# py-lidbox/lidbox

Hardware: AMD Instinct MI355X
Metric: utterances/sec (16kHz x 2s) log-mel + x-vector train step (higher is better)
Workload: dtype f32; 1 GPU; log-mel + x-vector 4-lang train step, bs=256 per GPU, fp32 (BASELINE configs[1]); reference_model=lidbox.models.xvector, global_batch=256, per_gpu_batch=256, samples_per_utt=32000, frames=198, mel=40, languages=4, optimizer=Adam(1e-3, eps=1e-7), parallelism=dp1, grad_buckets=1, grad_sync=none, hip_graph=True, resident_batches=4, feature_prefetch=False

## Files before the change

lidbox_amd/csrc/gemm.hip:

```cpp
#include <stdlib.h>

#include <atomic>

#include "gemm_shared.h"
#include "gemm_sk.h"
#include <string.h>
#include "gemm_dma.h"
#include "gemm_dma8.h"
#include "gemm_tuned.h"

namespace {

constexpr int BK = 16;
#define LBX_ROWS_BOUNDS(BM, BN) __launch_bounds__(256, ((BM) * (BN) >= 16384 ? 3 : ((BM) * (BN) >= 8192 ? 6 : 8)))
#define LBX_TN_BOUNDS(BM, BN) __launch_bounds__(256, ((BM) * (BN) >= 16384 ? 3 : 1))

template <int ROWS, bool ALIGNED, int NT = 256>
struct KInnerLoader {
    static constexpr int F4R = BK / 4;
    static constexpr int RPP = NT / F4R;
    static constexpr int PASSES = ROWS >= RPP ? ROWS / RPP : 1;
    static constexpr bool PARTIAL = ROWS < RPP;
    static constexpr int LD = ROWS + 8 / F4R;
    float4 v[PASSES];
    const float* ptr[PASSES];
    int c4, r0, k;

    __device__ __forceinline__ void init(const RowsD& rows, long row_base, long nrows, int tid, int kbeg) {
        c4 = tid % F4R;
        r0 = tid / F4R;
        k = kbeg + c4 * 4;
#pragma unroll
        for (int p = 0; p < PASSES; ++p) {
            const long r = row_base + r0 + p * RPP;
            ptr[p] = rows.base + ((r < nrows && !(PARTIAL && r0 >= ROWS)) ? row_offset(rows, (unsigned)r) : 0) + k;
        }
    }
    template <bool CHECK>
    __device__ __forceinline__ void load(int kend) {
#pragma unroll
        for (int p = 0; p < PASSES; ++p) {
            float4 x;
            if (!CHECK) {
                if (ALIGNED) x = *reinterpret_cast<const float4*>(ptr[p]);
                else x = make_float4(ptr[p][0], ptr[p][1], ptr[p][2], ptr[p][3]);
            } else {
                x = make_float4(0.f, 0.f, 0.f, 0.f);
                if (ALIGNED) {
                    if (k < kend) x = *reinterpret_cast<const float4*>(ptr[p]);
                } else {
                    if (k + 0 < kend) x.x = ptr[p][0];
                    if (k + 1 < kend) x.y = ptr[p][1];
                    if (k + 2 < kend) x.z = ptr[p][2];
                    if (k + 3 < kend) x.w = ptr[p][3];
                }
            }
            ptr[p] += BK;
            v[p] = x;
        }
        k += BK;
    }
    __device__ __forceinline__ void store(float* tile) const {
        if (PARTIAL && r0 >= ROWS) return;
#pragma unroll
        for (int p = 0; p < PASSES; ++p) {
            float* d = tile + (c4 * 4) * LD + r0 + p * RPP;
            d[0 * LD] = v[p].x;
            d[1 * LD] = v[p].y;
            d[2 * LD] = v[p].z;
            d[3 * LD] = v[p].w;
        }
    }
};

template <int COLS, bool ALIGNED, int NT = 256>
struct KOuterLoader {
    static constexpr int F4 = COLS / 4;
    static constexpr int RPP = NT / F4;
    static constexpr int PASSES = BK >= RPP ? BK / RPP : 1;
    static constexpr bool PARTIAL = BK < RPP;
    static constexpr int LD = COLS;
    float4 v[PASSES];
    const float* ptr[PASSES];
    long step;
    int c4, kk0, c, cload, kcur, ncols_;

    __device__ __forceinline__ void init(int tid, int col0, int ncols) {
        c4 = tid % F4;
        kk0 = tid / F4;
        if (PARTIAL && kk0 >= BK) kk0 -= BK;
        c = col0 + c4 * 4;
        ncols_ = ncols;
        cload = (ALIGNED && c >= ncols) ? 0 : c;
    }
    __device__ __forceinline__ void init_plain(const float* base, long ld, int kbeg, int col0, int ncols, int tid) {
        init(tid, col0, ncols);
        kcur = kbeg + kk0;
        step = (long)BK * ld;
#pragma unroll
        for (int p = 0; p < PASSES; ++p) ptr[p] = base + (long)(kcur + RPP * p) * ld + cload;
    }
    template <bool CHECK>
    __device__ __forceinline__ void load_plain(int kend) {
#pragma unroll
        for (int p = 0; p < PASSES; ++p) {
            v[p] = fetch<CHECK>(ptr[p], (kcur + RPP * p) < kend);
            ptr[p] += step;
        }
        kcur += BK;
    }
    template <bool CHECK>
    __device__ __forceinline__ void load_rows(const float* base, const long (&off)[PASSES],
                                              const bool (&ok)[PASSES]) {
#pragma unroll
        for (int p = 0; p < PASSES; ++p) v[p] = fetch<CHECK>(base + off[p] + cload, ok[p]);
    }
    template <bool CHECK>
    __device__ __forceinline__ float4 fetch(const float* src, bool row_ok) const {
        float4 x = make_float4(0.f, 0.f, 0.f, 0.f);
        if (ALIGNED) {
            if (!CHECK || row_ok) x = *reinterpret_cast<const float4*>(src);
        } else if (!CHECK || row_ok) {
            if (c + 0 < ncols_) x.x = src[0];
            if (c + 1 < ncols_) x.y = src[1];
            if (c + 2 < ncols_) x.z = src[2];
            if (c + 3 < ncols_) x.w = src[3];
        }
        return x;
    }
    __device__ __forceinline__ void store(float* tile) const {
#pragma unroll
        for (int p = 0; p < PASSES; ++p)
            *reinterpret_cast<float4*>(tile + (kk0 + RPP * p) * LD + c4 * 4) = v[p];
    }
};

template <int MI, int NJ, int LDA, int LDB>
__device__ __forceinline__ void mma_tile(const float* As, const float* Bs, int wm, int wn, int lane,
                                         f32x16 (&acc)[MI][NJ]) {
    const int h = lane >> 5, l = lane & 31;
    const float* ap = As + h * LDA + wm * (32 * MI) + l;
    const float* bp = Bs + h * LDB + wn * (32 * NJ) + l;
    float a[2][MI], b[2][NJ];
    __builtin_amdgcn_s_setprio(3);
#pragma unroll
    for (int i = 0; i < MI; ++i) a[0][i] = ap[32 * i];
#pragma unroll
    for (int j = 0; j < NJ; ++j) b[0][j] = bp[32 * j];
#pragma unroll
    for (int kk = 0; kk < BK; kk += 2) {
        const int cur = (kk >> 1) & 1, nxt = cur ^ 1;
        if (kk + 2 < BK) {
#pragma unroll
            for (int i = 0; i < MI; ++i) a[nxt][i] = ap[(kk + 2) * LDA + 32 * i];
#pragma unroll
            for (int j = 0; j < NJ; ++j) b[nxt][j] = bp[(kk + 2) * LDB + 32 * j];
        }
        __builtin_amdgcn_sched_barrier(0);
#pragma unroll
        for (int i = 0; i < MI; ++i)
#pragma unroll
            for (int j = 0; j < NJ; ++j)
// ... 232 lines not shown

__global__ void colsum_stage2(const float* __restrict__ partial, int slices, int N, float* __restrict__ out,
                              int accumulate) {
    const int c = blockIdx.x * blockDim.x + threadIdx.x;
    if (c >= N) return;
    float s = 0.f;
    for (int k = 0; k < slices; ++k) s += partial[(long)k * N + c];
    out[c] = accumulate ? out[c] + s : s;
}

inline bool sk_enabled() {
    const char* e = getenv("LIDBOX_GEMM_SK");
    return !(e && atoi(e) == 0);
}
inline unsigned sk_grid() {
    if (const char* e = getenv("LIDBOX_GEMM_SK_GRID")) {
        const int g = atoi(e);
        if (g >= 1 && g <= NUM_CU * SK_WGCU) return (unsigned)g;
    }
    return NUM_CU * SK_WGCU;
}
inline double sk_min_flop() {
    if (const char* e = getenv("LIDBOX_GEMM_SK_MIN_FLOP")) return atof(e);
    return 3.0e9;
}
constexpr int SK_MIN_SPAN = 8;
constexpr int SK_PART_STEPS = 16;

inline unsigned sk_next_epoch() {
    static std::atomic<unsigned> e{0};
    unsigned v;
    do v = e.fetch_add(1u) + 1u; while ((v & 0xffffffu) == 0u);
    return v & 0xffffffu;
}

struct SkRows {
    bool ok = false;
    SkPlan pl{};
    unsigned P = 0;
    size_t ws_need = 0;
};

inline bool sk_all() {
    const char* e = getenv("LIDBOX_GEMM_SK_ALL");
    return e && atoi(e) != 0;
}
inline bool sk_rows_policy(int kind, int K) { return sk_all() || (kind == 0 && K >= 1024); }
inline bool sk_tuned_out(int kind, long M, int N, int K) { return !sk_all() && tuned_gemm(kind, M, N, K) != nullptr; }

inline int skp_mode() {
    if (const char* e = getenv("LIDBOX_GEMM_SKP")) return atoi(e);
    return 1;
}

inline bool skp_policy(int kind, long M, int N, int K) {
    (void)kind; (void)M; (void)N; (void)K;
    return skp_mode() == 2;
}

SkRows sk_rows_plan(int kind, long M, int N, int K, bool pipelined = false) {
    SkRows c;
    if (!sk_enabled() || M < SK_BM || K % 4 != 0 || 2.0 * (double)M * N * K < sk_min_flop()) return c;
    if (!pipelined && !sk_rows_policy(kind, K)) return c;
    unsigned P = sk_grid();
    if (pipelined && P == (unsigned)(NUM_CU * SK_WGCU)) P = NUM_CU * SKP_WGCU;
    if (P % 8 != 0) return c;
    SkPlan& pl = c.pl;
    pl.tiles_n = (int)lbx_cdiv(N, SK_BN);
    const long T = lbx_cdiv(M, SK_BM) * pl.tiles_n;
    if (T > 0x3fffffffL) return c;
    pl.ntiles = (int)T;
    pl.nk = (int)lbx_cdiv(K, SK_BK);
    pl.ktail = K - (pl.nk - 1) * SK_BK;
    pl.dp_rounds = (int)(T / P);
    pl.sk_first = pl.dp_rounds * (int)P;
    pl.sk_tiles = (int)T - pl.sk_first;
    pl.parts = 0;
    if (pl.dp_rounds > 0 && pl.sk_tiles > 0) {
        long g = pl.nk / SK_PART_STEPS;
        if (g > (long)(P / 8) / lbx_cdiv(pl.sk_tiles, 8)) g = (long)(P / 8) / lbx_cdiv(pl.sk_tiles, 8);
        if (g < 1) g = 1;
        if (g > 200) g = 200;
        const long wg_cu = P / NUM_CU > 0 ? P / NUM_CU : 1;
        const double cu_parts = (double)pl.dp_rounds * pl.nk * wg_cu + (double)lbx_cdiv(pl.sk_tiles * g, NUM_CU) * ((double)pl.nk / g);
        const double cu_spans = 1.05 * (double)T * pl.nk / NUM_CU;
        if (cu_parts <= cu_spans) {
            pl.parts = (int)g;
        } else {
            --pl.dp_rounds;
            pl.sk_first = pl.dp_rounds * (int)P;
            pl.sk_tiles = (int)T - pl.sk_first;
        }
    }
    if (pl.parts == 0 && pl.sk_tiles > 0 && (long)pl.sk_tiles * pl.nk < (long)P * SK_MIN_SPAN) return c;
    if (pl.parts == 0 && pl.sk_tiles > 0 && (long)pl.nk * P / ((long)pl.sk_tiles * pl.nk) + 2 > 250) return c;
    if ((size_t)pl.sk_tiles * sizeof(unsigned) > SK_COUNTER_BYTES) return c;
    c.P = P;
    c.ws_need = SK_COUNTER_BYTES + (size_t)P * 2 * SK_SLAB * sizeof(float) + (pipelined ? SKP_DUMMY_BYTES : 0);
    c.ok = true;
    return c;
}

inline bool sk_extent_ok(const lidbox_rows_t& r, long cols) {
    const double last = (double)(r.batch > 0 ? r.batch - 1 : 0) * r.batch_stride + (double)(r.rows_per_batch > 0 ? r.rows_per_batch - 1 : 0) * r.row_stride + cols + 64;
    return last * 4.0 < 4.0e9;
}

inline bool sk_b_extent_ok(bool b_kinner, int K, int N, long ldb) {
    return ((double)(b_kinner ? N : K) + 16.0) * (double)ldb * 4.0 < 4.0e9;
}

void sk_set_lds_attr() {
    static const bool done = [] {
        (void)hipFuncSetAttribute((const void*)gemm_sk_rows_kernel<false>, hipFuncAttributeMaxDynamicSharedMemorySize, (int)SK_LDS_BYTES);
        (void)hipFuncSetAttribute((const void*)gemm_sk_rows_kernel<true>, hipFuncAttributeMaxDynamicSharedMemorySize, (int)SK_LDS_BYTES);
        (void)hipFuncSetAttribute((const void*)gemm_sk_tn_kernel, hipFuncAttributeMaxDynamicSharedMemorySize, (int)SK_LDS_BYTES);
#define LBX_SKP_ATTR(B_, M_, A_) (void)hipFuncSetAttribute((const void*)gemm_skp_rows_kernel<B_, M_, A_>, hipFuncAttributeMaxDynamicSharedMemorySize, (int)SKP_LDS_BYTES)
        LBX_SKP_ATTR(false, false, false); LBX_SKP_ATTR(false, true, false); LBX_SKP_ATTR(false, false, true); LBX_SKP_ATTR(false, true, true);
        LBX_SKP_ATTR(true, false, false); LBX_SKP_ATTR(true, true, false); LBX_SKP_ATTR(true, false, true); LBX_SKP_ATTR(true, true, true);
#undef LBX_SKP_ATTR
        return true;
    }();
    (void)done;
}

struct SkTn {
    bool ok = false;
    int splits = 0, tiles_n = 0, ntiles = 0;
    long rows_per_split = 0;
    size_t ws_need = 0;
};

SkTn sk_tn_plan(long M, int K1, int N) {
    SkTn c;
    if (!sk_enabled() || K1 % 4 != 0 || N % 4 != 0 || 2.0 * (double)M * N * K1 < 2.0 * sk_min_flop()) return c;
    c.tiles_n = (int)lbx_cdiv(N, SK_BN);
    c.ntiles = (int)lbx_cdiv(K1, SK_BM) * c.tiles_n;
    long g = (long)sk_grid() / c.ntiles;
    if (g < 1) g = 1;
    long rps = lbx_cdiv(lbx_cdiv(M, g), SK_BK) * SK_BK;
    if (rps < 8 * SK_BK) return c;
    if (rps > 8192) rps = 8192;
    c.rows_per_split = rps;
    c.splits = (int)lbx_cdiv(M, rps);
    c.ws_need = ((size_t)c.splits * K1 * N + (size_t)c.splits * N) * sizeof(float);
    c.ok = true;
    return c;
}

struct RowsChoice {
    int bm, bn, splits, k_per_split;
    bool no_tail_split = false;
    int waves = 4;
};

thread_local int g_last_launches[3] = {0, 0, 0};
thread_local int g_last_family = 0;
thread_local int g_first_tile[2] = {0, 0};
thread_local int g_last_carried = 0;

const int CAND[4][2] = {{128, 128}, {128, 64}, {64, 128}, {64, 64}};
const double TILE_EFF[4] = {1.0, 0.98, 0.97, 0.955};
const int RESIDENT[4] = {3, 4, 4, 6};
const double FIXED_STEPS[4] = {6.0, 5.0, 5.0, 3.0};

inline double conc_eff(double w) {
    if (w <= 1.0) return 0.55;
    if (w <= 2.0) return 0.55 + 0.25 * (w - 1.0);
    if (w <= 3.0) return 0.80 + 0.10 * (w - 2.0);
    return 0.92;
}

inline double launch_cost(int c, long wgs, double ksteps) {
    const int bm = CAND[c][0], bn = CAND[c][1];
    const double tile_t = (bm * bn / 16384.0) * (ksteps + FIXED_STEPS[c]) / TILE_EFF[c];
    double per_cu = (double)lbx_cdiv(wgs, NUM_CU);
    if (wgs > NUM_CU && wgs % NUM_CU != 0) {
        const double fluid = (double)wgs / NUM_CU + 0.12;
        if (fluid < per_cu) per_cu = fluid;
    }
    const double conc = per_cu < RESIDENT[c] ? (double)wgs / NUM_CU : (double)RESIDENT[c];
    return per_cu * tile_t / conc_eff(conc < 1.0 ? 1.0 : conc);
}

RowsChoice choose_rows(int kind, long M, int N, int K, size_t ws_bytes) {
    if (const TunedGemm* t = tuned_gemm(kind, M, N, K)) {
        const int kps = (int)(lbx_cdiv(lbx_cdiv(K, t->splits), BK) * BK);
        const int splits = (int)lbx_cdiv(K, kps);
        if (splits == 1 || (size_t)splits * M * N * sizeof(float) <= ws_bytes)
            return RowsChoice{t->bm, t->bn, splits, kps, t->no_tail_split != 0, (t->waves == 8 && t->bm == 128) ? 8 : 4};
    }
    RowsChoice best{128, 128, 1, K};
    double best_cost = 1e30;
    for (int c = 0; c < 4; ++c) {
        const int bm = CAND[c][0], bn = CAND[c][1];
        const long tiles = lbx_cdiv(M, bm) * lbx_cdiv(N, bn);
        for (int s = 1; s <= 64; s *= 2) {
            int kps = (int)(lbx_cdiv(lbx_cdiv(K, s), BK) * BK);
            const int splits = (int)lbx_cdiv(K, kps);
            if (s > 1 && (splits < 2 || kps < 4 * BK)) break;
            if (splits > 1 && (size_t)splits * M * N * sizeof(float) > ws_bytes) break;
            double cost = launch_cost(c, tiles * splits, (double)kps / BK);
            if (splits > 1) cost += 5.0 + (double)M * N * 4.0 * (splits + 1) / 3.0e6;
            if (cost < best_cost) { best_cost = cost; best = RowsChoice{bm, bn, splits, kps}; }
            if (splits < s) break;
        }
    }
    return best;
}

RowsChoice choose_rows_env(int kind, long M, int N, int K, size_t wsb) {
    RowsChoice ch = choose_rows(kind, M, N, K, wsb);
    if (M >= 4096) {
        if (const char* f = getenv(kind == 1 ? "LIDBOX_GEMM_NT8" : "LIDBOX_GEMM_NN8")) {
            const int bn = atoi(f);
            if (bn == 64 || bn == 128) return RowsChoice{128, bn, 1, K, false, 8};
        }
    }
    if (const char* f = getenv("LIDBOX_GEMM_PLAN")) {
        int bm = 0, bn = 0, sp = 0, wv = 4;
        if (sscanf(f, "%d,%d,%d,%d", &bm, &bn, &sp, &wv) >= 3 && (bm == 64 || bm == 128) && (bn == 64 || bn == 128) && sp >= 1) {
            const int kps = (int)(lbx_cdiv(lbx_cdiv(K, sp), BK) * BK);
            const int splits = (int)lbx_cdiv(K, kps);
            if (splits == 1 || (size_t)splits * M * N * sizeof(float) <= wsb)
                ch = RowsChoice{bm, bn, splits, kps, false, (wv == 8 && bm == 128) ? 8 : 4};
        }
    }
    return ch;
}

template <int BM, int BN, bool B_KINNER>
void launch_rows8_t(bool al, dim3 grid, hipStream_t st, RowsD Ad, const float* Bm, long ldb, RowsOutD Co, float* P,
                    long m_beg, long m_end, int K, int N, int epi, const float* aux, int tiles_n, unsigned ntiles, int kps) {
    if (al)
        hipLaunchKernelGGL((gemm_rows8_kernel<BM, BN, B_KINNER, true>), grid, dim3(512), 0, st, Ad, Bm, ldb, Co, P, m_beg,
                           m_end, K, N, epi, aux, tiles_n, ntiles, kps);
    else
        hipLaunchKernelGGL((gemm_rows8_kernel<BM, BN, B_KINNER, false>), grid, dim3(512), 0, st, Ad, Bm, ldb, Co, P, m_beg,
                           m_end, K, N, epi, aux, tiles_n, ntiles, kps);
}

template <int BM, int BN, bool B_KINNER>
void launch_rows_t(bool al, dim3 grid, hipStream_t st, RowsD Ad, const float* Bm, long ldb, RowsOutD Co, float* P,
                   long m_beg, long m_end, int K, int N, int epi, const float* aux, int tiles_n, unsigned ntiles, int kps) {
    if (al)
        hipLaunchKernelGGL((gemm_rows_kernel<BM, BN, B_KINNER, true>), grid, dim3(256), 0, st, Ad, Bm, ldb, Co, P, m_beg,
                           m_end, K, N, epi, aux, tiles_n, ntiles, kps);
    else
        hipLaunchKernelGGL((gemm_rows_kernel<BM, BN, B_KINNER, false>), grid, dim3(256), 0, st, Ad, Bm, ldb, Co, P, m_beg,
                           m_end, K, N, epi, aux, tiles_n, ntiles, kps);
}

inline int dma_mode() {
    if (const char* e = getenv("LIDBOX_GEMM_DMA")) return atoi(e);
    return 1;
}

template <int BM, int BN, bool B_KINNER>
void launch_rows_dma_t(dim3 grid, hipStream_t st, RowsD Ad, const float* Bm, long ldb, RowsOutD Co, float* P, long m_beg, long m_end,
                       int K, int N, int epi, const float* aux, int tiles_n, unsigned ntiles, int kps, const DmaStream& sp, const ReduceJobs& rj) {
    hipLaunchKernelGGL((gemm_rows_dma_kernel<BM, BN, B_KINNER>), grid, dim3(256), 0, st, Ad, Bm, ldb, Co, P, m_beg, m_end, K, N, epi,
                       aux, tiles_n, ntiles, kps, sp, rj);
}

inline long carry_cap() {
    if (const char* e = getenv("LIDBOX_GEMM_CARRY_BLOCKS")) { const long v = atol(e); if (v >= 8) return v; }
    return 96;
}
struct Carry {
    const ReduceJob* jobs = nullptr;
    int njobs = 0;
    bool carried = false;
};

constexpr int DMA_STREAM_MIN_STEPS = 8;
constexpr int DMA_STREAM_MAX_G = 8;
struct DmaStreamPlan {
    int g = 0;
    long whole = 0, rem = 0;
    size_t ws_need = 0;
};
inline DmaStreamPlan dma_stream_plan(int bm, int bn, long M, int N, int K) {
    DmaStreamPlan pl;
    int force = -1;
    if (const char* e = getenv("LIDBOX_GEMM_STREAM_TAIL")) force = atoi(e);
    if (force == 0) return pl;
    const long tiles = lbx_cdiv(M, bm) * lbx_cdiv(N, bn);
    const long rem = tiles % NUM_CU;
    if (tiles < NUM_CU || rem == 0) return pl;
    const int nk = (int)lbx_cdiv(K, SK_BK);
    int best = 1;
    double best_cost = 1.0;
    for (int g = 2; g <= DMA_STREAM_MAX_G && nk / g >= DMA_STREAM_MIN_STEPS; ++g) {
        const double cost = (double)lbx_cdiv(rem * g, (long)NUM_CU) / g + 0.03 + 0.01 * g;
        if (cost < best_cost - 1e-9) { best_cost = cost; best = g; }
    }
    if (force > 1 && nk / force >= 2 && force <= 64) best = force;
    else if (best_cost > 0.9) return pl;
    if (best < 2) return pl;
    pl.g = best; pl.rem = rem; pl.whole = tiles - rem;
    pl.ws_need = SK_COUNTER_BYTES + (size_t)rem * best * bm * bn * sizeof(float);
    return pl;
}

template <bool B_KINNER>
int launch_rows_range(const RowsChoice& ch, bool al, RowsD Ad, const float* Bm, long ldb, RowsOutD Co, long m_beg,
                      long m_end, int K, int N, int epi, const float* aux, float* P, hipStream_t st, bool dma_ok = false,
                      const DmaStreamPlan* stream = nullptr, void* ws = nullptr, Carry* carry = nullptr) {
    const long Msub = m_end - m_beg;
    if (Msub <= 0) return LIDBOX_OK;
    const int tiles_n = (int)lbx_cdiv(N, ch.bn);
    const long ntiles = lbx_cdiv(Msub, ch.bm) * tiles_n;
    dim3 grid((unsigned)ntiles, (unsigned)ch.splits);
    if (g_last_launches[0] == 0) { g_first_tile[0] = ch.bm; g_first_tile[1] = ch.bn; }
    ++g_last_launches[(ch.bm == g_first_tile[0] && ch.bn == g_first_tile[1]) ? 0 : 1];
    if (ch.splits > 1) ++g_last_launches[2];
#define LBX_ROWS(BM_, BN_) launch_rows_t<BM_, BN_, B_KINNER>(al, grid, st, Ad, Bm, ldb, Co, P, m_beg, m_end, K, N, epi, aux, tiles_n, (unsigned)ntiles, ch.k_per_split)
#define LBX_ROWS8(BM_, BN_) launch_rows8_t<BM_, BN_, B_KINNER>(al, grid, st, Ad, Bm, ldb, Co, P, m_beg, m_end, K, N, epi, aux, tiles_n, (unsigned)ntiles, ch.k_per_split)
#define LBX_ROWS_DMA(BM_, BN_) launch_rows_dma_t<BM_, BN_, B_KINNER>(grid, st, Ad, Bm, ldb, Co, P, m_beg, m_end, K, N, epi, aux, tiles_n, ntiles_k, ch.k_per_split, sp, rj)
    if (dma_ok && al && dma_mode() != 0) {
        g_last_family = 1;
        DmaStream sp;
        const bool dma8 = ch.waves == 8 && ch.bm == 128;
        ReduceJobs rj;
        if (carry && !carry->carried && carry->njobs > 0) {
            rj = pack_carry(carry->jobs, carry->njobs, carry_cap());
            carry->carried = rj.total > 0;
        }
        unsigned ntiles_k = (unsigned)ntiles;
        if (stream && stream->g > 1 && ch.splits == 1) {
            sp.pieces = (unsigned)(stream->rem * stream->g);
            sp.npad = (sp.pieces + 7u) & ~7u;
            sp.g = stream->g;
            sp.first_tile = (unsigned)stream->whole;
            sp.epoch = sk_next_epoch();
            sp.counters = (unsigned*)ws;
            sp.slabs = (float*)((char*)ws + SK_COUNTER_BYTES);
            ntiles_k = (unsigned)stream->whole;
            grid.x = sp.npad + ntiles_k;
        }
        grid.x += rj.total;
        if (dma8) {
            g_last_family = 3;
            if (ch.bn == 128)
                hipLaunchKernelGGL((gemm_rows_dma8_kernel<128, B_KINNER>), grid, dim3(512), 0, st, Ad, Bm, ldb, Co, P, m_beg, m_end, K, N, epi, aux, tiles_n,
                                   ntiles_k, ch.k_per_split, sp, rj);
            else
                hipLaunchKernelGGL((gemm_rows_dma8_kernel<64, B_KINNER>), grid, dim3(512), 0, st, Ad, Bm, ldb, Co, P, m_beg, m_end, K, N, epi, aux, tiles_n,
                                   ntiles_k, ch.k_per_split, sp, rj);
        } else
        if (ch.bm == 128 && ch.bn == 128) LBX_ROWS_DMA(128, 128);
        else if (ch.bm == 128) LBX_ROWS_DMA(128, 64);
        else if (ch.bn == 128) LBX_ROWS_DMA(64, 128);
        else LBX_ROWS_DMA(64, 64);
    } else
    if (ch.waves == 8 && ch.bm == 128 && ch.bn == 128) LBX_ROWS8(128, 128);
    else if (ch.waves == 8 && ch.bm == 128 && ch.bn == 64) LBX_ROWS8(128, 64);
    else if (ch.bm == 128 && ch.bn == 128) LBX_ROWS(128, 128);
    else if (ch.bm == 128) LBX_ROWS(128, 64);
    else if (ch.bn == 128) LBX_ROWS(64, 128);
    else LBX_ROWS(64, 64);
#undef LBX_ROWS
#undef LBX_ROWS8
    LBX_LAUNCH_OK();
    if (ch.splits > 1) {
        long g = lbx_cdiv(Msub * N, 256);
        if (g > 2048) g = 2048;
        hipLaunchKernelGGL(rows_reduce_kernel, dim3((unsigned)g), dim3(256), 0, st, (const float*)P, ch.splits, m_beg,
                           Msub, N, Co, epi, aux);
        LBX_LAUNCH_OK();
    }
    return LIDBOX_OK;
}

inline int cand_index(int bm, int bn) { return bm == 128 ? (bn == 128 ? 0 : 1) : (bn == 128 ? 2 : 3); }

template <bool B_KINNER>
int launch_rows(lidbox_rows_t A, const float* Bm, long ldb, lidbox_rows_out_t Cd, int K, int N, int epi,
                const float* aux, void* ws, size_t ws_bytes, hipStream_t st, Carry* carry = nullptr) {
    const long M = (long)A.batch * A.rows_per_batch;
    g_last_launches[0] = g_last_launches[1] = g_last_launches[2] = 0;
    g_last_family = 0;
    if (M == 0 || N == 0) return LIDBOX_OK;
    const size_t wsb = ws ? ws_bytes : 0;
    const RowsChoice ch = choose_rows_env(B_KINNER ? 1 : 0, M, N, K, wsb);
    const bool al = rows_aligned(A) && K % 4 == 0 && aligned16(Bm) && ldb % 4 == 0 &&
                    (B_KINNER ? true : N % 4 == 0);
    RowsD Ad = to_dev(A);
    RowsOutD Co{Cd.base, Cd.batch_stride, Cd.row_stride, Cd.batch, Cd.rows_per_batch};
    float* P = (float*)ws;

    if (al && !getenv("LIDBOX_GEMM_PLAN") && aligned16(ws) && !sk_tuned_out(B_KINNER ? 1 : 0, M, N, K) &&
        sk_b_extent_ok(B_KINNER, K, N, ldb)) {
        const bool has_mask_ = epi == LIDBOX_EPI_RELU_MASK || epi == LIDBOX_EPI_ACCUM_RELU_MASK;
        const bool skp_ok = skp_mode() != 0 && (Cd.batch == 1 || Cd.rows_per_batch >= 32) && N % 4 == 0 && aligned16(Cd.base) &&
                            Cd.row_stride % 4 == 0 && (Cd.batch == 1 || Cd.batch_stride % 4 == 0) && (!has_mask_ || aligned16(aux)) &&
                            skp_policy(B_KINNER ? 1 : 0, M, N, K);
        if (skp_ok) {
            const SkRows sk = sk_rows_plan(B_KINNER ? 1 : 0, M, N, K, true);
            if (sk.ok && wsb >= sk.ws_need && sk_extent_ok(A, K)) {
                sk_set_lds_attr();
                g_last_launches[0] = 1;
                g_last_family = 2;
                g_first_tile[0] = SK_BM; g_first_tile[1] = SK_BN;
                unsigned* counters = (unsigned*)ws;
                float* slabs = (float*)((char*)ws + SK_COUNTER_BYTES);
                float* dummy = slabs + (size_t)sk.P * 2 * SK_SLAB;
                const bool has_mask = epi == LIDBOX_EPI_RELU_MASK || epi == LIDBOX_EPI_ACCUM_RELU_MASK;
                const bool accum = epi == LIDBOX_EPI_ACCUM || epi == LIDBOX_EPI_ACCUM_RELU_MASK || epi == LIDBOX_EPI_ACCUM_RELU;
                const unsigned ep = sk_next_epoch();
#define LBX_SKP(MASK_, ACC_)                                                                                                \
    hipLaunchKernelGGL((gemm_skp_rows_kernel<B_KINNER, MASK_, ACC_>), dim3(sk.P), dim3(256), (MASK_ || ACC_) ? SKP_LDS_BYTES : SK_LDS_BYTES, st, Ad, Bm, ldb, Co, M, K, \
                       N, epi, aux, sk.pl, ep, counters, slabs, dummy)
                if (has_mask && accum) LBX_SKP(true, true);
                else if (has_mask) LBX_SKP(true, false);
                else if (accum) LBX_SKP(false, true);
                else LBX_SKP(false, false);
#undef LBX_SKP
                LBX_LAUNCH_OK();
                return LIDBOX_OK;
            }
        }
        const SkRows sk = sk_rows_plan(B_KINNER ? 1 : 0, M, N, K);
        if (sk.ok && wsb >= sk.ws_need && sk_extent_ok(A, K)) {
            sk_set_lds_attr();
            g_last_launches[0] = 1;
            g_last_family = 2;
            g_first_tile[0] = SK_BM; g_first_tile[1] = SK_BN;
            unsigned* counters = (unsigned*)ws;
            float* slabs = (float*)((char*)ws + SK_COUNTER_BYTES);
            hipLaunchKernelGGL((gemm_sk_rows_kernel<B_KINNER>), dim3(sk.P), dim3(256), SK_LDS_BYTES, st, Ad, Bm, ldb, Co, M, K, N, epi,
                               aux, sk.pl, sk_next_epoch(), counters, slabs);
            LBX_LAUNCH_OK();
            return LIDBOX_OK;
        }
    }

    const bool dma_ok = al && sk_extent_ok(A, K) && sk_b_extent_ok(B_KINNER, K, N, ldb);
    if (dma_ok && dma_mode() != 0 && ch.splits == 1 && aligned16(ws)) {
        const DmaStreamPlan spl = dma_stream_plan(ch.bm, ch.bn, M, N, K);
        if (spl.g > 1 && wsb >= spl.ws_need)
            return launch_rows_range<B_KINNER>(ch, al, Ad, Bm, ldb, Co, 0, M, K, N, epi, aux, P, st, dma_ok, &spl, ws, carry);
    }
    const bool no_tail_split = ch.no_tail_split || getenv("LIDBOX_GEMM_NO_TAIL_SPLIT") != nullptr;
    if (!no_tail_split && ch.splits == 1) {
        const int tiles_n = (int)lbx_cdiv(N, ch.bn);
        const long tiles_m = lbx_cdiv(M, ch.bm);
        const long wgs = tiles_m * tiles_n;
        const long rounds = wgs / NUM_CU;
        if (rounds >= 1 && wgs % NUM_CU != 0) {
            const long main_tiles_m = rounds * NUM_CU / tiles_n;
            const long m_main = main_tiles_m * ch.bm;
            const long m_rem = M - m_main;
            if (main_tiles_m >= 1 && m_rem > 0) {
                const RowsChoice rem = choose_rows(B_KINNER ? 1 : 0, m_rem, N, K, wsb);
                const int c = cand_index(ch.bm, ch.bn), cr = cand_index(rem.bm, rem.bn);
                const double ksteps = (double)lbx_cdiv(K, BK);
                const double whole = launch_cost(c, wgs, ksteps);
                double split = launch_cost(c, main_tiles_m * tiles_n, ksteps) + 4.0 +
                               launch_cost(cr, lbx_cdiv(m_rem, rem.bm) * lbx_cdiv(N, rem.bn) * rem.splits,
                                           (double)rem.k_per_split / BK);
                if (rem.splits > 1) split += 5.0 + (double)m_rem * N * 4.0 * (rem.splits + 1) / 3.0e6;
                if (split < 0.97 * whole) {
                    int rc = launch_rows_range<B_KINNER>(ch, al, Ad, Bm, ldb, Co, 0, m_main, K, N, epi, aux, P, st, dma_ok, nullptr, nullptr, carry);
                    if (rc) return rc;
                    return launch_rows_range<B_KINNER>(rem, al, Ad, Bm, ldb, Co, m_main, M, K, N, epi, aux, P, st, dma_ok);
                }
            }
        }
    }
    return launch_rows_range<B_KINNER>(ch, al, Ad, Bm, ldb, Co, 0, M, K, N, epi, aux, P, st, dma_ok, nullptr, nullptr, carry);
}

struct TnPlan {
    int bm, bn, splits;
    long rows_per_split;
};

TnPlan tn_plan(long M, int K1, int N) {
    if (const char* f = getenv("LIDBOX_GEMM_TN_PLAN")) {
        int bm = 0, bn = 0;
        long sp = 0;
        if (sscanf(f, "%d,%d,%ld", &bm, &bn, &sp) == 3 && (bm == 64 || bm == 128) && (bn == 64 || bn == 128) && sp >= 1) {
            const long rps = lbx_cdiv(lbx_cdiv(M, sp), BK) * BK;
            return TnPlan{bm, bn, (int)lbx_cdiv(M, rps), rps};
        }
    }
    if (const TunedGemm* t = tuned_gemm(2, M, N, K1)) {
        const long rps = lbx_cdiv(lbx_cdiv(M, (long)t->splits), BK) * BK;
        return TnPlan{t->bm, t->bn, (int)lbx_cdiv(M, rps), rps};
    }
    TnPlan best{128, 128, 1, M};
    double best_cost = 1e30;
    for (int c = 0; c < 4; ++c) {
        const int bm = CAND[c][0], bn = CAND[c][1];
        const long tiles = lbx_cdiv(K1, bm) * lbx_cdiv(N, bn);
        for (long target = NUM_CU; target <= 8 * NUM_CU; target += NUM_CU / 2) {
            long s = target / tiles;
            if (s < 1) s = 1;
            const long max_s = lbx_cdiv(M, 4 * BK);
            if (s > max_s) s = max_s;
            if (s < 1) s = 1;
            long rps = lbx_cdiv(lbx_cdiv(M, s), BK) * BK;
            s = lbx_cdiv(M, rps);
            double cost = launch_cost(c, tiles * s, (double)rps / BK);
            cost += 5.0 + (double)K1 * N * 4.0 * (s + 1) / 3.0e6;
            if (cost < best_cost) { best_cost = cost; best = TnPlan{bm, bn, (int)s, rps}; }
        }
    }
    return best;
}

template <int BM, int BN>
void launch_tn_t(bool al, unsigned grid, hipStream_t st, RowsD A, RowsD Bd, float* P, float* Pc, long M, int K1, int N,
                 int tiles_n, int ntiles, long rps) {
    if (al)
        hipLaunchKernelGGL((gemm_tn_kernel<BM, BN, true>), dim3(grid), dim3(256), 0, st, A, Bd, P, Pc, M, K1, N, tiles_n,
                           ntiles, rps);
    else
        hipLaunchKernelGGL((gemm_tn_kernel<BM, BN, false>), dim3(grid), dim3(256), 0, st, A, Bd, P, Pc, M, K1, N, tiles_n,
                           ntiles, rps);
}

}

extern "C" int lidbox_gemm_plan_query(int kind, long M, int N, int K, size_t workspace_bytes, int* out4) {
    LBX_ARG(out4 && M > 0 && N > 0 && K > 0 && kind >= 0 && kind <= 2, "kind in {0 nn, 1 nt, 2 tn}, positive sizes");
    if (kind == 2) {
        const TnPlan pl = tn_plan(M, K, N);
        out4[0] = pl.bm; out4[1] = pl.bn; out4[2] = pl.splits; out4[3] = (int)pl.rows_per_split;
    } else {
        const RowsChoice ch = choose_rows_env(kind, M, N, K, workspace_bytes);
        out4[0] = ch.bm; out4[1] = ch.bn; out4[2] = ch.splits; out4[3] = ch.k_per_split;
    }
    return LIDBOX_OK;
}

extern "C" int lidbox_gemm_plan_is_stream_k(int kind, long M, int N, int K, size_t workspace_bytes) {
    if (M <= 0 || N <= 0 || K <= 0 || kind < 0 || kind > 2) return 0;
    if (kind == 2) {
        const SkTn t = sk_tn_plan(M, K, N);
        return t.ok && workspace_bytes >= t.ws_need && !sk_tuned_out(2, M, N, K);
    }
    {
        const SkRows r = sk_rows_plan(kind, M, N, K);
        return r.ok && workspace_bytes >= r.ws_need && (kind == 1 || N % 4 == 0) && !sk_tuned_out(kind, M, N, K);
    }
    return LIDBOX_OK;
}

extern "C" int lidbox_gemm_plan_waves(int kind, long M, int N, int K, size_t workspace_bytes) {
    if (M <= 0 || N <= 0 || K <= 0 || kind < 0 || kind > 1) return 4;
    return choose_rows_env(kind, M, N, K, workspace_bytes).waves;
}

extern "C" int lidbox_gemm_last_family(void) { return g_last_family; }

extern "C" int lidbox_gemm_plan_stream_tail(int kind, long M, int N, int K, size_t workspace_bytes) {
    if (M <= 0 || N <= 0 || K <= 0 || kind < 0 || kind > 1 || dma_mode() == 0) return 0;
    if (!getenv("LIDBOX_GEMM_PLAN") && lidbox_gemm_plan_is_stream_k(kind, M, N, K, workspace_bytes)) return 0;
    const RowsChoice ch = choose_rows_env(kind, M, N, K, workspace_bytes);
    if (ch.splits != 1) return 0;
    const DmaStreamPlan spl = dma_stream_plan(ch.bm, ch.bn, M, N, K);
    return (spl.g > 1 && workspace_bytes >= spl.ws_need) ? spl.g : 0;
}

extern "C" int lidbox_gemm_last_launches(int* out3) {
    LBX_ARG(out3, "out3 != NULL");
    out3[0] = g_last_launches[0]; out3[1] = g_last_launches[1]; out3[2] = g_last_launches[2];
    return LIDBOX_OK;
}

extern "C" size_t lidbox_gemm_rows_workspace(long M, int N, int K) {
    if (M <= 0 || N <= 0 || K <= 0) return 0;
    size_t need = 0;
    for (int kind = 0; kind < 2; ++kind) {
        const RowsChoice ch = choose_rows(kind, M, N, K, (size_t)64 << 20);
        if (ch.splits > 1 && (size_t)ch.splits * M * N * sizeof(float) > need) need = (size_t)ch.splits * M * N * sizeof(float);
    }
    for (int bm = 64; bm <= 128; bm += 64)
        for (int bn = 64; bn <= 128; bn += 64) {
            const DmaStreamPlan spl = dma_stream_plan(bm, bn, M, N, K);
            if (spl.g > 1 && spl.ws_need > need) need = spl.ws_need;
        }
    for (int kind = 0; kind < 2; ++kind) {
        const SkRows sk = sk_rows_plan(kind, M, N, K);
        if (sk.ok && sk.ws_need > need) need = sk.ws_need;
        if (skp_mode() != 0 && skp_policy(kind, M, N, K)) {
            const SkRows skp = sk_rows_plan(kind, M, N, K, true);
            if (skp.ok && skp.ws_need > need) need = skp.ws_need;
        }
    }
    return need;
}

extern "C" int lidbox_gemm_nn(lidbox_rows_t A, const float* Bm, long ldb, lidbox_rows_out_t C, int K, int N,
                              int epilogue, const float* aux, void* workspace, size_t workspace_bytes,
                              lidbox_stream_t stream) {
    if (validate_rows_call(__func__, A, Bm, ldb, C, K, N, epilogue, aux, N)) return LIDBOX_E_INVALID;
    return launch_rows<false>(A, Bm, ldb, C, K, N, epilogue, aux, workspace, workspace_bytes, (hipStream_t)stream);
}


extern "C" int lidbox_gemm_nt(lidbox_rows_t A, const float* Bm, long ldb, lidbox_rows_out_t C, int K, int N,
                              int epilogue, const float* aux, void* workspace, size_t workspace_bytes,
                              lidbox_stream_t stream) {
    if (validate_rows_call(__func__, A, Bm, ldb, C, K, N, epilogue, aux, K)) return LIDBOX_E_INVALID;
    return launch_rows<true>(A, Bm, ldb, C, K, N, epilogue, aux, workspace, workspace_bytes, (hipStream_t)stream);
}

extern "C" size_t lidbox_gemm_tn_workspace(int M, int K1, int N) {
    if (M <= 0 || K1 <= 0 || N <= 0) return 0;
    const TnPlan pl = tn_plan(M, K1, N);
    size_t need = ((size_t)pl.splits * K1 * N + (size_t)pl.splits * N) * sizeof(float);
    const SkTn sk = sk_tn_plan(M, K1, N);
    if (sk.ok && sk.ws_need > need) need = sk.ws_need;
    return need;
}

namespace {

int tn_partial_launch(const char* fn, lidbox_rows_t A, lidbox_rows_t Bd, float* Cm, long ldc, int K1, int N, int accumulate,
                      float* bias_grad, void* workspace, size_t workspace_bytes, hipStream_t st, ReduceJob* job) {
    *job = ReduceJob{};
    if (check_rows(fn, A.base, A.batch_stride, A.row_stride, A.batch, A.rows_per_batch)) return LIDBOX_E_INVALID;
    if (check_rows(fn, Bd.base, Bd.batch_stride, Bd.row_stride, Bd.batch, Bd.rows_per_batch)) return LIDBOX_E_INVALID;
    LBX_ARG(Cm && K1 >= 1 && N >= 1 && ldc >= N, "C != NULL, K1, N >= 1, ldc >= N");
    const long M = (long)A.batch * A.rows_per_batch;
    LBX_ARG(M == (long)Bd.batch * Bd.rows_per_batch, "A and B row counts differ");
    LBX_ARG(M >= 1, "M >= 1");
    auto finish = [&](const float* P, const float* Pc, int splits) {
        const long n = (long)K1 * N;
        if (reduce_job_vec_ok(P, Pc, splits, n, N, Cm, ldc, bias_grad)) *job = make_reduce_job(P, Pc, splits, n, N, Cm, ldc, accumulate, bias_grad);
        else launch_splitk_reduce(P, Pc, splits, n, N, Cm, ldc, accumulate, bias_grad, st);
    };
    {
        const SkTn sk = sk_tn_plan(M, K1, N);
        if (sk.ok && !getenv("LIDBOX_GEMM_TN_PLAN") && !sk_tuned_out(2, M, N, K1) && workspace && aligned16(workspace) && workspace_bytes >= sk.ws_need &&
            rows_aligned(A) && rows_aligned(Bd) && sk_extent_ok(A, K1) && sk_extent_ok(Bd, N)) {
            sk_set_lds_attr();
            g_last_launches[0] = 1; g_last_launches[1] = 0; g_last_launches[2] = 1;
            g_last_family = 2;
            float* P = (float*)workspace;
            float* Pc = bias_grad ? P + (size_t)sk.splits * K1 * N : nullptr;
            hipLaunchKernelGGL(gemm_sk_tn_kernel, dim3((unsigned)(sk.ntiles * sk.splits)), dim3(256), SK_LDS_BYTES, st, to_dev(A),
                               to_dev(Bd), P, Pc, M, K1, N, sk.tiles_n, sk.ntiles, sk.rows_per_split);
            LBX_LAUNCH_OK();
            finish(P, Pc, sk.splits);
            LBX_LAUNCH_OK();
            return LIDBOX_OK;
        }
    }
    const TnPlan pl = tn_plan(M, K1, N);
    const size_t need = ((size_t)pl.splits * K1 * N + (size_t)pl.splits * N) * sizeof(float);
    LBX_ARG(workspace && workspace_bytes >= need, "workspace too small (lidbox_gemm_tn_workspace)");
    g_last_launches[0] = 1; g_last_launches[1] = 0; g_last_launches[2] = 1;
    g_last_family = 0;
    const int tiles_n = (int)lbx_cdiv(N, pl.bn);
    const int ntiles = (int)(lbx_cdiv(K1, pl.bm) * tiles_n);
    const bool al = rows_aligned(A) && rows_aligned(Bd) && K1 % 4 == 0 && N % 4 == 0;
    float* P = (float*)workspace;
    float* Pc = bias_grad ? P + (size_t)pl.splits * K1 * N : nullptr;
    const unsigned grid = (unsigned)(ntiles * pl.splits);
    if (al && dma_mode() != 0 && sk_extent_ok(A, K1) && sk_extent_ok(Bd, N) && pl.rows_per_split % SK_BK == 0) {
        g_last_family = 1;
#define LBX_TN_DMA(BM_, BN_) hipLaunchKernelGGL((gemm_tn_dma_kernel<BM_, BN_>), dim3(grid), dim3(256), 0, st, to_dev(A), to_dev(Bd), P, Pc, M, K1, N, tiles_n, ntiles, pl.rows_per_split)
        if (pl.bm == 128 && pl.bn == 128) LBX_TN_DMA(128, 128);
        else if (pl.bm == 128) LBX_TN_DMA(128, 64);
        else if (pl.bn == 128) LBX_TN_DMA(64, 128);
        else LBX_TN_DMA(64, 64);
#undef LBX_TN_DMA
        LBX_LAUNCH_OK();
        finish(P, Pc, pl.splits);
        LBX_LAUNCH_OK();
        return LIDBOX_OK;
    }
#define LBX_TN(BM_, BN_) launch_tn_t<BM_, BN_>(al, grid, st, to_dev(A), to_dev(Bd), P, Pc, M, K1, N, tiles_n, ntiles, pl.rows_per_split)
    if (pl.bm == 128 && pl.bn == 128) LBX_TN(128, 128);
    else if (pl.bm == 128) LBX_TN(128, 64);
    else if (pl.bn == 128) LBX_TN(64, 128);
    else LBX_TN(64, 64);
#undef LBX_TN
    LBX_LAUNCH_OK();
    finish(P, Pc, pl.splits);
    LBX_LAUNCH_OK();
    return LIDBOX_OK;
}

static_assert(sizeof(lidbox_reduce_job_t) == sizeof(ReduceJob), "lidbox_reduce_job_t mirrors ReduceJob");
inline ReduceJob job_in(const lidbox_reduce_job_t* j) {
    ReduceJob r;
    if (j) memcpy(&r, j, sizeof r);
    return r;
}
inline int jobs_in(const lidbox_reduce_job_t* jobs, int njobs, ReduceJob (&out)[MAX_CARRY]) {
    int m = 0;
    for (int i = 0; jobs && i < njobs; ++i) {
        if (jobs[i].nblocks == 0) continue;
        if (m == MAX_CARRY) return -1;
        out[m++] = job_in(jobs + i);
    }
    return m;
}

int run_reduce_jobs(const ReduceJob* jobs, int njobs, hipStream_t st) {
    ReduceJobs js;
    for (int i = 0, m = 0; i < njobs && m < MAX_CARRY; ++i) {
        if (jobs[i].nblocks == 0) continue;
        js.j[m++] = jobs[i];
        js.total += jobs[i].nblocks;
    }
    if (js.total == 0) return LIDBOX_OK;
    hipLaunchKernelGGL(splitk_reduce4_kernel, dim3(js.total), dim3(256), 0, st, js);
    LBX_LAUNCH_OK();
    return LIDBOX_OK;
}

}

extern "C" int lidbox_gemm_tn(lidbox_rows_t A, lidbox_rows_t Bd, float* Cm, long ldc, int K1, int N,
                              int accumulate, float* bias_grad, void* workspace, size_t workspace_bytes,
                              lidbox_stream_t stream) {
    ReduceJob job;
    int rc = tn_partial_launch(__func__, A, Bd, Cm, ldc, K1, N, accumulate, bias_grad, workspace, workspace_bytes, (hipStream_t)stream, &job);
    if (rc) return rc;
    return run_reduce_jobs(&job, 1, (hipStream_t)stream);
}

extern "C" int lidbox_gemm_tn_partial(lidbox_rows_t A, lidbox_rows_t Bd, float* Cm, long ldc, int K1, int N, int accumulate,
                                      float* bias_grad, void* workspace, size_t workspace_bytes, lidbox_reduce_job_t* job,
// ... 210 lines not shown
```

Before: 120,700 utterances/s.

## Add MFMA small-GEMM kernel with in-block K-split for listed small shapes

Adds a dedicated small-M GEMM path that gives each 32x32 output tile one workgroup of 16 waves. Each wave takes a slice of K, runs fp32 MFMA 32x32x2 with buffer loads and an LDS-swizzled A stage, and the waves reduce partial sums in LDS before the epilogue. It is selected only for an allow-listed shape (NN, 256x512x512) where the classic planner would have chosen a split-K launch. The aim is to avoid the split-K workspace round trip and its separate reduce kernel. The trade-off is a large LDS reduction buffer per block and a fixed tile shape that may use the GPU poorly.

New measurement: 121,100 utterances/s, median of 6. Within noise of the previous version (+0.3%).

```diff
diff --git a/lidbox_amd/csrc/gemm.hip b/lidbox_amd/csrc/gemm.hip
--- a/lidbox_amd/csrc/gemm.hip
+++ b/lidbox_amd/csrc/gemm.hip
@@ -8,6 +8,7 @@
 #include "gemm_dma.h"
 #include "gemm_dma8.h"
 #include "gemm_tuned.h"
+#include "gemm_small.h"
 
 namespace {
 
@@ -546,6 +547,7 @@
     int bm, bn, splits, k_per_split;
     bool no_tail_split = false;
     int waves = 4;
+    bool small = false;
 };
 
 thread_local int g_last_launches[3] = {0, 0, 0};
@@ -577,7 +579,7 @@
     return per_cu * tile_t / conc_eff(conc < 1.0 ? 1.0 : conc);
 }
 
-RowsChoice choose_rows(int kind, long M, int N, int K, size_t ws_bytes) {
+RowsChoice choose_rows_classic(int kind, long M, int N, int K, size_t ws_bytes) {
     if (const TunedGemm* t = tuned_gemm(kind, M, N, K)) {
         const int kps = (int)(lbx_cdiv(lbx_cdiv(K, t->splits), BK) * BK);
         const int splits = (int)lbx_cdiv(K, kps);
@@ -603,8 +605,18 @@
     return best;
 }
 
-RowsChoice choose_rows_env(int kind, long M, int N, int K, size_t wsb) {
-    RowsChoice ch = choose_rows(kind, M, N, K, wsb);
+RowsChoice choose_rows(int kind, long M, int N, int K, size_t ws_bytes, bool allow_small = true) {
+    const RowsChoice ch = choose_rows_classic(kind, M, N, K, ws_bytes);
+    if (allow_small && small_listed(kind, M, N, K, ch.splits > 1)) {
+        RowsChoice sm{SMALL_T, SMALL_T, 1, K};
+        sm.small = true;
+        return sm;
+    }
+    return ch;
+}
+
+RowsChoice choose_rows_env(int kind, long M, int N, int K, size_t wsb, bool allow_small = true) {
+    RowsChoice ch = choose_rows(kind, M, N, K, wsb, allow_small);
     if (M >= 4096) {
         if (const char* f = getenv(kind == 1 ? "LIDBOX_GEMM_NT8" : "LIDBOX_GEMM_NN8")) {
             const int bn = atoi(f);
@@ -777,7 +789,18 @@
     g_last_family = 0;
     if (M == 0 || N == 0) return LIDBOX_OK;
     const size_t wsb = ws ? ws_bytes : 0;
-    const RowsChoice ch = choose_rows_env(B_KINNER ? 1 : 0, M, N, K, wsb);
+    RowsChoice ch = choose_rows_env(B_KINNER ? 1 : 0, M, N, K, wsb);
+    if (ch.small) {
+        if (small_operands_ok(B_KINNER, A, Bm, ldb, Cd, M, N, K)) {
+            g_last_launches[0] = 1;
+            g_last_family = 4;
+            g_first_tile[0] = g_first_tile[1] = SMALL_T;
+            launch_small<B_KINNER>(A, Bm, ldb, Cd, M, N, K, epi, aux, st);
+            LBX_LAUNCH_OK();
+            return LIDBOX_OK;
+        }
+        ch = choose_rows_env(B_KINNER ? 1 : 0, M, N, K, wsb, false);
+    }
     const bool al = rows_aligned(A) && K % 4 == 0 && aligned16(Bm) && ldb % 4 == 0 &&
                     (B_KINNER ? true : N % 4 == 0);
     RowsD Ad = to_dev(A);
@@ -847,7 +870,7 @@
             const long m_main = main_tiles_m * ch.bm;
             const long m_rem = M - m_main;
             if (main_tiles_m >= 1 && m_rem > 0) {
-                const RowsChoice rem = choose_rows(B_KINNER ? 1 : 0, m_rem, N, K, wsb);
+                const RowsChoice rem = choose_rows(B_KINNER ? 1 : 0, m_rem, N, K, wsb, false);
                 const int c = cand_index(ch.bm, ch.bn), cr = cand_index(rem.bm, rem.bn);
                 const double ksteps = (double)lbx_cdiv(K, BK);
                 const double whole = launch_cost(c, wgs, ksteps);
@@ -969,7 +992,7 @@
     if (M <= 0 || N <= 0 || K <= 0) return 0;
     size_t need = 0;
     for (int kind = 0; kind < 2; ++kind) {
-        const RowsChoice ch = choose_rows(kind, M, N, K, (size_t)64 << 20);
+        const RowsChoice ch = choose_rows(kind, M, N, K, (size_t)64 << 20, false);
         if (ch.splits > 1 && (size_t)ch.splits * M * N * sizeof(float) > need) need = (size_t)ch.splits * M * N * sizeof(float);
     }
     for (int bm = 64; bm <= 128; bm += 64)
diff --git a/lidbox_amd/csrc/gemm_small.h b/lidbox_amd/csrc/gemm_small.h
--- /dev/null
+++ b/lidbox_amd/csrc/gemm_small.h
@@ -0,0 +1,181 @@
+#pragma once
+#include "gemm_shared.h"
+
+namespace {
+
+constexpr int SMALL_T = 32;
+constexpr int SMALL_W = 16;
+constexpr int SMALL_UNIT = 8;
+constexpr int SMALL_UB = 4;
+constexpr long SMALL_MAX_M = 1024;
+
+struct SmallGemm {
+    int kind;
+    long M;
+    int N, K;
+};
+const SmallGemm SMALL_GEMM[] = {
+    {0, 256, 512, 512},
+};
+
+inline bool small_listed(int kind, long M, int N, int K, bool would_split) {
+    if (kind < 0 || kind > 1 || M > SMALL_MAX_M || getenv("LIDBOX_GEMM_NO_SMALL")) return false;
+    if (const char* e = getenv("LIDBOX_GEMM_SMALL_ALL")) { if (atoi(e) != 0) return true; }
+    if (!would_split) return false;
+    for (const SmallGemm& s : SMALL_GEMM)
+        if (s.kind == kind && s.M == M && s.N == N && s.K == K) return true;
+    return false;
+}
+
+inline bool small_operands_ok(bool b_kinner, const lidbox_rows_t& A, const float* Bm, long ldb, const lidbox_rows_out_t& C, long M, int N, int K) {
+    return M >= 1 && M <= SMALL_MAX_M && A.batch == 1 && C.batch == 1 && aligned16(A.base) && A.row_stride % 4 == 0 &&
+           (double)M * (double)A.row_stride * 4.0 < 4.0e9 && (double)(b_kinner ? N : K) * (double)ldb * 4.0 < 4.0e9 &&
+           (!b_kinner || (aligned16(Bm) && ldb % 4 == 0));
+}
+
+template <bool B_KINNER>
+__global__ __launch_bounds__(SMALL_W * 64) void gemm_small_kernel(const float* __restrict__ A, long lda, const float* __restrict__ Bm, long ldb,
+                                                                  float* C, long ldc, int M, int N, int K, int epi, const float* aux,
+                                                                  int tiles_m, unsigned ntiles) {
+    __shared__ float red[SMALL_W * 16 * 64];
+    const int lane = threadIdx.x & 63, w = __builtin_amdgcn_readfirstlane((int)(threadIdx.x >> 6));
+    const int l = lane & 31, h = lane >> 5;
+    unsigned tile = blockIdx.x;
+    if ((ntiles & 7u) == 0u) tile = (blockIdx.x & 7u) * (ntiles >> 3) + (blockIdx.x >> 3);
+    const int tile_n = (int)(tile / (unsigned)tiles_m), tile_m = (int)(tile - (unsigned)tile_n * (unsigned)tiles_m);
+    const int m0 = tile_m * SMALL_T, n0 = tile_n * SMALL_T;
+    const int arow = m0 + l < M ? m0 + l : M - 1;
+    const int bcol = n0 + l < N ? n0 + l : N - 1;
+    const float* Ap = A + (long)arow * lda;
+    const float* Bp = B_KINNER ? Bm + (long)bcol * ldb : Bm + bcol;
+
+    const int units = (K + SMALL_UNIT - 1) / SMALL_UNIT;
+    const int upw = (units + SMALL_W - 1) / SMALL_W;
+    const int kbeg = w * upw * SMALL_UNIT;
+    int kend = kbeg + upw * SMALL_UNIT;
+    if (kend > K) kend = K;
+
+    typedef float f4 __attribute__((ext_vector_type(4)));
+    float* As = red + w * (SMALL_T * 32);
+    const int srow = lane >> 3, schunk = lane & 7;
+    const __amdgpu_buffer_rsrc_t ra = __builtin_amdgcn_make_buffer_rsrc(const_cast<float*>(A), 0, 0xffffffffu, 0x00020000);
+    const __amdgpu_buffer_rsrc_t rb = __builtin_amdgcn_make_buffer_rsrc(const_cast<float*>(Bm), 0, 0xffffffffu, 0x00020000);
+    unsigned va[4];
+#pragma unroll
+    for (int t = 0; t < 4; ++t) {
+        const int r = m0 + srow + 8 * t;
+        va[t] = (unsigned)(((long)(r < M ? r : M - 1) * lda + 4 * schunk) * 4);
+    }
+    const unsigned vb = B_KINNER ? (unsigned)(((long)bcol * ldb + 4 * h) * 4) : (unsigned)(((long)(4 * h) * ldb + bcol) * 4);
+    const unsigned ldb4 = (unsigned)(ldb * 4);
+    auto load_a = [&](f4 (&g)[4], int k0) {
+#pragma unroll
+        for (int t = 0; t < 4; ++t) g[t] = __builtin_bit_cast(f4, __builtin_amdgcn_raw_buffer_load_b128(ra, va[t], (unsigned)k0 * 4u, 0));
+    };
+    auto stage_a = [&](const f4 (&g)[4], float (&fa)[SMALL_UB][4]) {
+#pragma unroll
+        for (int t = 0; t < 4; ++t) *reinterpret_cast<f4*>(As + (srow + 8 * t) * 32 + 4 * (schunk ^ srow)) = g[t];
+        wave_lds_sync();
+#pragma unroll
+        for (int u = 0; u < SMALL_UB; ++u) {
+            const f4 av = *reinterpret_cast<const f4*>(As + l * 32 + 4 * ((2 * u + h) ^ (l & 7)));
+            fa[u][0] = av.x; fa[u][1] = av.y; fa[u][2] = av.z; fa[u][3] = av.w;
+        }
+        wave_lds_sync();
+    };
+    auto load_b = [&](float (&fb)[SMALL_UB][4], int k0) {
+#pragma unroll
+        for (int u = 0; u < SMALL_UB; ++u) {
+            const unsigned k = (unsigned)(k0 + u * SMALL_UNIT);
+            if (B_KINNER) {
+                const f4 bv = __builtin_bit_cast(f4, __builtin_amdgcn_raw_buffer_load_b128(rb, vb, k * 4u, 0));
+                fb[u][0] = bv.x; fb[u][1] = bv.y; fb[u][2] = bv.z; fb[u][3] = bv.w;
+            } else {
+#pragma unroll
+                for (int j = 0; j < 4; ++j)
+                    fb[u][j] = __builtin_bit_cast(float, __builtin_amdgcn_raw_buffer_load_b32(rb, vb, (k + (unsigned)j) * ldb4, 0));
+            }
+        }
+    };
+    auto load_edge = [&](float (&fa)[SMALL_UB][4], float (&fb)[SMALL_UB][4], int k0) {
+#pragma unroll
+        for (int u = 0; u < SMALL_UB; ++u)
+#pragma unroll
+            for (int j = 0; j < 4; ++j) {
+                const int k = k0 + u * SMALL_UNIT + 4 * h + j;
+                const bool ok = k < kend;
+                const int kc = ok ? k : K - 1;
+                const float av = Ap[kc];
+                const float bv = B_KINNER ? Bp[kc] : Bp[(long)kc * ldb];
+                fa[u][j] = ok ? av : 0.f;
+                fb[u][j] = ok ? bv : 0.f;
+            }
+    };
+    f32x16 acc;
+#pragma unroll
+    for (int r = 0; r < 16; ++r) acc[r] = 0.f;
+    auto mma = [&](const float (&fa)[SMALL_UB][4], const float (&fb)[SMALL_UB][4]) {
+#pragma unroll
+        for (int u = 0; u < SMALL_UB; ++u)
+#pragma unroll
+            for (int j = 0; j < 4; ++j) acc = __builtin_amdgcn_mfma_f32_32x32x2f32(fa[u][j], fb[u][j], acc, 0, 0, 0);
+    };
+    constexpr int BATCH = SMALL_UB * SMALL_UNIT;
+    const int nfull = kend > kbeg ? (kend - kbeg) / BATCH : 0;
+    float fa[SMALL_UB][4], fb0[SMALL_UB][4], fb1[SMALL_UB][4];
+    if (nfull > 0) {
+        f4 g[4];
+        load_a(g, kbeg);
+        load_b(fb0, kbeg);
+        int i = 0;
+        for (; i + 2 <= nfull; i += 2) {
+            stage_a(g, fa);
+            load_a(g, kbeg + (i + 1) * BATCH);
+            load_b(fb1, kbeg + (i + 1) * BATCH);
+            __builtin_amdgcn_sched_barrier(0);
+            mma(fa, fb0);
+            __builtin_amdgcn_sched_barrier(0);
+            stage_a(g, fa);
+            const int k2 = kbeg + (i + 2 < nfull ? i + 2 : nfull - 1) * BATCH;
+            load_a(g, k2);
+            load_b(fb0, k2);
+            __builtin_amdgcn_sched_barrier(0);
+            mma(fa, fb1);
+            __builtin_amdgcn_sched_barrier(0);
+        }
+        if (i < nfull) {
+            stage_a(g, fa);
+            mma(fa, fb0);
+        }
+    }
+    const int ktail = kbeg + nfull * BATCH;
+    if (ktail < kend) {
+        load_edge(fa, fb0, ktail);
+        mma(fa, fb0);
+    }
+    __syncthreads();
+
+#pragma unroll
+    for (int r = 0; r < 16; ++r) red[(w * 16 + r) * 64 + lane] = acc[r];
+    __syncthreads();
+    float s = red[w * 64 + lane];
+#pragma unroll
+    for (int ww = 1; ww < SMALL_W; ++ww) s += red[(ww * 16 + w) * 64 + lane];
+    const int row = m0 + (w & 3) + 8 * (w >> 2) + 4 * h, col = n0 + l;
+    if (row < M && col < N) {
+        const long idx = (long)row * ldc + col;
+        const float bias = (epi == LIDBOX_EPI_BIAS || epi == LIDBOX_EPI_BIAS_RELU) ? aux[col] : 0.f;
+        C[idx] = apply_epi(s, epi, bias, aux, idx, C + idx);
+    }
+}
+
+template <bool B_KINNER>
+inline void launch_small(const lidbox_rows_t& A, const float* Bm, long ldb, const lidbox_rows_out_t& C, long M, int N, int K, int epi,
+                         const float* aux, hipStream_t st) {
+    const int tiles_m = (int)lbx_cdiv(M, (long)SMALL_T);
+    const unsigned ntiles = (unsigned)(tiles_m * lbx_cdiv((long)N, (long)SMALL_T));
+    hipLaunchKernelGGL((gemm_small_kernel<B_KINNER>), dim3(ntiles), dim3(SMALL_W * 64), 0, st, A.base, A.row_stride, Bm, ldb, C.base,
+                       C.row_stride, (int)M, N, K, epi, aux, tiles_m, ntiles);
+}
+
+}
```
